# tensorlayer/HyperPose

Hardware: AMD Instinct MI355X
Metric: end-to-end FPS (preproc+DNN+PAF parse) @ 368x432 (higher is better)
Workload: dtype f32; 1 GPU; configs[1]: Lightweight-OpenPose (MobilenetDilated) + PAF parser, batch 8 @ 368x432 per GPU; frames from pinned host memory (one H2D per batch), parser on the network's own maps, humans to the host; key=configs[1]/f32, global_batch=8, parallelism=frame-sharded x1, no steady-state collective, pipes_per_gpu=4, parser_input=the network's own heat-maps

## Files before the change

hyperpose_amd/csrc/conv32_winograd.hip:

```cpp
#include "conv_fp32.hpp"

#include "conv32_epilogue.hpp"
#include "conv_device.hpp"

#include <cstdlib>
#include <vector>

namespace hp {

namespace {

typedef float f32x4 __attribute__((ext_vector_type(4)));
typedef __attribute__((address_space(1))) float gfloat;
typedef __attribute__((address_space(1))) f32x4 gf32x4;

constexpr int WCK = 16;
constexpr int HALO_W = 10;
constexpr int RAW_PB = WCK * 4;
constexpr int VP = 24 * 4;

template <int MW, int NC = 2>
struct wino_geom {
    static constexpr int NT = 64 * MW;
    static constexpr int TB = 4 * NC;
    static constexpr int HALO_H = 8 * NC + 2;
    static constexpr int PATCH_H = HALO_H + 1;
    static constexpr int RAW_Q = PATCH_H * HALO_W * 4;
    static constexpr int NQ = (RAW_Q + NT - 1) / NT;
    static constexpr int RAW_BYTES = NQ * NT * 16;
    static constexpr int NI = 4 * NC / MW;
    static_assert(NI >= 1, "a transform item per wavefront");
    static constexpr int TMS = MW / 2;
    static constexpr int SLAB_PITCH = rows_geom<TMS>::PITCH, SLAB_BYTES = 64 * NC * SLAB_PITCH * 4;
    static constexpr int VPOS = 16 * NC * VP, VBUF = 16 * VPOS;
    static constexpr int LDS_BYTES = RAW_BYTES + (VBUF > SLAB_BYTES ? VBUF : SLAB_BYTES);
    static constexpr int PVPOS = 16 * NC * 64, PVBUF = 16 * PVPOS;
    static constexpr int PLDS_BYTES = RAW_BYTES + (2 * PVBUF > SLAB_BYTES ? 2 * PVBUF : SLAB_BYTES);
};

__device__ __forceinline__ long tvw_off(const tview32& t, int b, int y, int x)
{
    return ((long)b * t.img + (long)y * t.wp + x) * t.cs + t.coff;
}

}

template <int MW, bool PIPE, int NC = 2>
__global__ __launch_bounds__(64 * MW, MW == 8 ? 1 : NC == 1 ? 3 : 2) void conv32_winograd_kernel(const conv32_params p, int tiles_x, int tiles_y, int vh, int T)
{
    static_assert(!PIPE || MW == 4, "the pipelined form is the four-wavefront one");
    using G = wino_geom<MW, NC>;
    constexpr int NT = G::NT, NQ = G::NQ, SLAB_PITCH = G::SLAB_PITCH, VPOS = G::VPOS;
    extern __shared__ __attribute__((aligned(16))) unsigned char lds[];
    unsigned char* const raw = lds;
    unsigned char* const vb = lds + G::RAW_BYTES;

    const int tid = threadIdx.x, lane = tid & 63, wave = tid >> 6;
    const int NG = p.Cout_pad / (16 * MW), ntiles = tiles_x * tiles_y * (vh || T ? 1 : p.B);
    const int Hin = vh ? (p.B - 1) * vh + p.H : p.H;
    const int bj = blockIdx.x >> 3, by = bj % NG;
    int t = (bj / NG) * 8 + (blockIdx.x & 7);
    if (t >= ntiles)
        return;
    const int bx = t;
    const int tx = t % tiles_x;
    t /= tiles_x;
    const int ty = t % tiles_y, b = t / tiles_y;
    const int y0 = ty * (8 * NC), x0 = tx * 8;
    const int MT = p.Cout_pad / 16, mt = by * MW + wave;
    const int nch = p.Cin / WCK;
    int dbg_i = 0;
#define HP_STAMP()                                                     \
    if (p.dbg && bx == 1 && by == 0 && tid == 0)       \
        p.dbg[dbg_i++] = __builtin_amdgcn_s_memtime();
    HP_STAMP();
    if (p.dbg && bx == 1 && by == 0 && tid == 0)
        p.dbg[119] = __builtin_readcyclecounter(), p.dbg[120] = __builtin_amdgcn_s_memrealtime();

    int kb = G::TB, sh = 0, img0 = b, ly0 = y0 - 1, l0 = 0;
    if (T) {
        const int r0 = ty * G::TB;
        img0 = r0 / T, l0 = r0 - img0 * T, ly0 = 2 * l0 - 1;
        kb = min(T - l0, G::TB), sh = kb < G::TB && !(p.H & 1);
    }
    const int Hlim = T ? p.H : Hin, ylow = kb < G::TB ? 2 * kb + 1 + sh : G::PATCH_H;
    const int nvalid = (G::HALO_H + sh) * HALO_W * 4;
    long goff[NQ];
    bool qok[NQ];
#pragma unroll
    for (int i = 0; i < NQ; ++i) {
        const int q = min(tid + i * NT, nvalid - 1);
        const int hp = q >> 2, c4 = q & 3;
        const int hy = hp / HALO_W, hx = hp - hy * HALO_W;
        const bool below = hy >= ylow;
        const int bi = below ? img0 + 1 : img0, y = below ? hy - ylow : ly0 + hy, x = x0 - 1 + hx;
        qok[i] = y <= Hlim && x <= p.W && bi < p.B;
        goff[i] = tvw_off(p.in, min(bi, p.B - 1), min(y, Hlim), min(x, p.W)) + c4 * 4;
    }
    f32x4 stage[NQ];
    auto gload = [&](int c) {
#pragma unroll
        for (int i = 0; i < NQ; ++i)
            stage[i] = *reinterpret_cast<const f32x4*>(p.in.p + goff[i] + min(c, nch - 1) * WCK);
    };
    auto to_lds = [&]() {
#pragma unroll
        for (int i = 0; i < NQ; ++i)
            *reinterpret_cast<f32x4*>(raw + (tid + i * NT) * 16) = qok[i] ? stage[i] : f32x4{ 0.f, 0.f, 0.f, 0.f };
    };
    auto tile_src = [&](int tile, int quad) {
        const int tr = tile >> 2;
        return raw + ((2 * tr + (tr >= kb ? sh : 0)) * HALO_W + 2 * (tile & 3)) * RAW_PB + quad * 16;
    };
    auto transform = [&]() {
#pragma unroll
        for (int k = 0; k < G::NI; ++k) {
            const int item = wave + k * MW, i = NC == 2 ? item >> 1 : item;
            const int quad = lane >> 4, tile = (NC == 2 ? (item & 1) * 16 : 0) + (lane & 15);
            const int ra = i == 0 ? 0 : i == 2 ? 2 : 1, rb = i == 0 ? 2 : i == 1 ? 2 : i == 2 ? 1 : 3;
            const float sg = i == 1 ? 1.f : -1.f;
            const unsigned char* const src = tile_src(tile, quad);
            f32x4 Td[4];
#pragma unroll
            for (int j = 0; j < 4; ++j) {
                const f32x4 a = *reinterpret_cast<const f32x4*>(src + (ra * HALO_W + j) * RAW_PB);
                const f32x4 bq = *reinterpret_cast<const f32x4*>(src + (rb * HALO_W + j) * RAW_PB);
                Td[j] = a + sg * bq;
            }
            constexpr int PS = PIPE ? G::PVPOS : VPOS;
            unsigned char* const dst = PIPE ? vb + (i * 4) * PS + tile * 64 + ((quad ^ ((4 - (tile >> 2)) & 3)) * 16) : vb + (i * 4) * PS + tile * VP + quad * 16;
            *reinterpret_cast<f32x4*>(dst) = Td[0] - Td[2];
            *reinterpret_cast<f32x4*>(dst + PS) = Td[1] + Td[2];
            *reinterpret_cast<f32x4*>(dst + 2 * PS) = Td[2] - Td[1];
            *reinterpret_cast<f32x4*>(dst + 3 * PS) = Td[1] - Td[3];
        }
    };
    f32x4 ta[4], tb[4];
    auto transform_piece = [&](int pos, int buf) {
        const int k = pos >> 3, ps = pos & 7;
        if (k >= G::NI)
            return;
        const int item = wave + k * MW, i = NC == 2 ? item >> 1 : item;
        const int quad = lane >> 4, tile = (NC == 2 ? (item & 1) * 16 : 0) + (lane & 15);
        const int ra = i == 0 ? 0 : i == 2 ? 2 : 1, rb = i == 0 ? 2 : i == 1 ? 2 : i == 2 ? 1 : 3;
        const unsigned char* const src = tile_src(tile, quad);
        if (ps < 4) {
            ta[ps] = *reinterpret_cast<const f32x4*>(src + (ra * HALO_W + ps) * RAW_PB);
            tb[ps] = *reinterpret_cast<const f32x4*>(src + (rb * HALO_W + ps) * RAW_PB);
        } else {
            if (ps == 4) {
                const float sg = i == 1 ? 1.f : -1.f;
#pragma unroll
                for (int j = 0; j < 4; ++j)
                    ta[j] = ta[j] + sg * tb[j];
            }
            unsigned char* const dst = vb + buf * G::PVBUF + (i * 4 + (ps - 4)) * G::PVPOS + tile * 64 + ((quad ^ ((4 - (tile >> 2)) & 3)) * 16);
            *reinterpret_cast<f32x4*>(dst) = ps == 4 ? ta[0] - ta[2] : ps == 5 ? ta[1] + ta[2] : ps == 6 ? ta[2] - ta[1] : ta[1] - ta[3];
        }
    };

    const long step_stride = (long)MT * 256;
    const float* const wp = p.w_wino + (long)mt * 256 + lane * 4;
    const int nsteps = nch * 16;
    constexpr int RING = PIPE ? 4 : 8, AHEAD = PIPE ? 3 : 6;
    f32x4 fa[RING];
    auto aload = [&](int slot, int s) { fa[slot] = *reinterpret_cast<const f32x4*>(wp + (long)min(s, nsteps - 1) * step_stride); };

    f32x4 acc[16][NC];
#pragma unroll
    for (int i = 0; i < 16; ++i)
#pragma unroll
        for (int nc = 0; nc < NC; ++nc)
            acc[i][nc] = f32x4{ 0.f, 0.f, 0.f, 0.f };

    const int btile = lane & 15, kq = lane >> 4;
    const unsigned char* const vsrc = PIPE ? vb + btile * 64 + ((kq ^ ((4 - (btile >> 2)) & 3)) * 16) : vb + btile * VP + kq * 16;
    constexpr int BPOS = PIPE ? G::PVPOS : VPOS, BNT = PIPE ? 16 * 64 : 16 * VP;

    gload(0);
    if constexpr (PIPE) {
#pragma unroll
        for (int a = 0; a < AHEAD; ++a)
            aload(a, a);
        to_lds();
        gload(1);
        lds_barrier();
        HP_STAMP();
        transform();
        lds_barrier();
        to_lds();
        gload(2);
        lds_barrier();
        HP_STAMP();
    } else {
#pragma unroll
        for (int a = 0; a < AHEAD; ++a)
            aload(a, a);
    }
    int s = 0;
#pragma unroll 1
    for (int c = 0; c < nch; ++c) {
        if constexpr (!PIPE) {
            to_lds();
            gload(c + 1);
            lds_barrier();
            HP_STAMP();
            transform();
            lds_barrier();
            HP_STAMP();
        }
        const unsigned char* const vcur = vsrc + (PIPE ? (c & 1) * G::PVBUF : 0);
        f32x4 fb[2][NC];
#pragma unroll
        for (int nc = 0; nc < NC; ++nc)
            fb[0][nc] = *reinterpret_cast<const f32x4*>(vcur + nc * BNT);
#pragma unroll
        for (int pos = 0; pos < 16; ++pos) {
            const int cur = pos & 1, npos = pos + 1 < 16 ? pos + 1 : pos;
#pragma unroll
            for (int nc = 0; nc < NC; ++nc)
                fb[cur ^ 1][nc] = *reinterpret_cast<const f32x4*>(vcur + npos * BPOS + nc * BNT);
            aload((pos + AHEAD) % RING, s + AHEAD);
            const int slot = pos % RING;
#pragma unroll
            for (int e = 0; e < 4; ++e)
#pragma unroll
                for (int nc = 0; nc < NC; ++nc)
                    acc[pos][nc] = __builtin_amdgcn_mfma_f32_16x16x4f32(fa[slot][e], fb[cur][nc][e], acc[pos][nc], 0, 0, 0);
            if constexpr (PIPE)
                transform_piece(pos, (c + 1) & 1);
            __builtin_amdgcn_sched_group_barrier(0x008, 1, 0);
            __builtin_amdgcn_sched_group_barrier(0x100, 1, 0);
            if constexpr (NC == 2) {
                __builtin_amdgcn_sched_group_barrier(0x008, 1, 0);
                __builtin_amdgcn_sched_group_barrier(0x100, 1, 0);
            }
            __builtin_amdgcn_sched_group_barrier(0x008, 1, 0);
            __builtin_amdgcn_sched_group_barrier(0x020, 1, 0);
            __builtin_amdgcn_sched_group_barrier(0x008, NC == 2 ? 5 : 2, 0);
            __builtin_amdgcn_sched_barrier(0);
            ++s;
        }
        HP_STAMP();
        if constexpr (PIPE) {
            if (c + 1 < nch) {
                lds_barrier();
                to_lds();
                gload(c + 3);
                lds_barrier();
                HP_STAMP();
            }
        }
    }

    int tid_o = tid;
    asm volatile("" : "+v"(tid_o));
    const int lane_o = tid_o & 63, btile_o = lane_o & 15, kq_o = lane_o >> 4;
    using R = rows_geom<G::TMS>;
    constexpr int RPW = 64 * NC / MW, NPASS = RPW / R::RPP;
    static_assert(RPW % R::RPP == 0, "slab rows per pass");
    const int dc4 = lane_o % R::LPR, dm = by * 16 * MW + dc4 * 4;
    const bool dany = dm < p.Cout, quads = (p.Cout & 3) == 0;
    const bool out_vec = quads && ((p.out.coff | p.out.cs) & 3) == 0, res_vec = quads && ((p.res.coff | p.res.cs) & 3) == 0;
    const int dmc = dany ? dm : 0;
    int dpix[NPASS], rpix[NPASS];
    bool dok[NPASS];
#pragma unroll
    for (int k = 0; k < NPASS; ++k) {
        const int rr = wave * RPW + k * R::RPP + lane_o / R::LPR, ab = rr / (16 * NC), tile = rr % (16 * NC), tr = tile >> 2;
        const int ox = x0 + 2 * (tile & 3) + (ab & 1);
        int oy, ob;
        if (T)
            ob = tr >= kb ? img0 + 1 : img0, oy = 2 * (tr >= kb ? tr - kb : l0 + tr) + (ab >> 1);
        else {
            oy = y0 + 2 * tr + (ab >> 1);
            ob = vh ? oy / vh : b, oy -= vh ? ob * vh : 0;
        }
        dok[k] = oy < p.OH && ox < p.OW && ob < p.B && dany;
        const int oyc = min(oy, p.OH - 1), oxc = min(ox, p.OW - 1), obc = min(ob, p.B - 1);
        dpix[k] = (obc * p.out.img + oyc * p.out.wp) + oxc;
        rpix[k] = (obc * p.res.img + oyc * p.res.wp) + oxc;
    }
    f32x4 dres[NPASS];
#pragma unroll
    for (int k = 0; k < NPASS; ++k)
        dres[k] = f32x4{ 0.f, 0.f, 0.f, 0.f };
    const gfloat* const gres = (const gfloat*)p.res.p;
    gfloat* const gout = (gfloat*)p.out.p;
    if (gres) {
        if (res_vec) {
#pragma unroll
            for (int k = 0; k < NPASS; ++k)
                dres[k] = *reinterpret_cast<const gf32x4*>(gres + ((long)rpix[k] * p.res.cs + p.res.coff + dmc));
        } else {
#pragma unroll
            for (int k = 0; k < NPASS; ++k)
#pragma unroll
                for (int e = 0; e < 4; ++e)
                    dres[k][e] = gres[(long)rpix[k] * p.res.cs + p.res.coff + min(dm + e, p.Cout - 1)];
        }
    }
    const f32x4 dbs = *(const gf32x4*)(p.bias + dm);
    f32x4 dsl = { p.act_slope, p.act_slope, p.act_slope, p.act_slope };
    if (p.alpha)
        dsl = *(const gf32x4*)(p.alpha + dm);
    lds_barrier();
    HP_STAMP();
    float* const slab = reinterpret_cast<float*>(vb);
#pragma unroll
    for (int nt = 0; nt < NC; ++nt) {
        f32x4 S[2][4];
#pragma unroll
        for (int j = 0; j < 4; ++j) {
            S[0][j] = acc[j][nt] + acc[4 + j][nt] + acc[8 + j][nt];
            S[1][j] = acc[4 + j][nt] - acc[8 + j][nt] - acc[12 + j][nt];
        }
#pragma unroll
        for (int a = 0; a < 2; ++a) {
            const f32x4 y0v = S[a][0] + S[a][1] + S[a][2], y1v = S[a][1] - S[a][2] - S[a][3];
            *reinterpret_cast<f32x4*>(slab + ((a * 2 + 0) * (16 * NC) + nt * 16 + btile_o) * SLAB_PITCH + wave * 16 + kq_o * 4) = y0v;
            *reinterpret_cast<f32x4*>(slab + ((a * 2 + 1) * (16 * NC) + nt * 16 + btile_o) * SLAB_PITCH + wave * 16 + kq_o * 4) = y1v;
        }
    }
    HP_STAMP();
    lds_barrier();
    HP_STAMP();
    const float* const wslab = slab + (wave * RPW + lane_o / R::LPR) * SLAB_PITCH + dc4 * 4;
    f32x4 dv[NPASS];
#pragma unroll
    for (int k = 0; k < NPASS; ++k)
        dv[k] = *reinterpret_cast<const f32x4*>(wslab + k * R::RPP * SLAB_PITCH);
#pragma unroll
    for (int k = 0; k < NPASS; ++k) {
        f32x4 o;
#pragma unroll
        for (int e = 0; e < 4; ++e) {
            float x = dv[k][e] + dbs[e];
            if (p.res.p && p.res_before_act)
                x += dres[k][e];
            x = x > 0.f ? fminf(x, p.act_hi) : x * dsl[e];
            if (p.res.p && !p.res_before_act)
                x += dres[k][e];
            o[e] = x;
        }
        dv[k] = o;
    }
    if (out_vec) {
#pragma unroll
        for (int k = 0; k < NPASS; ++k)
            if (dok[k])
                *reinterpret_cast<gf32x4*>(gout + ((long)dpix[k] * p.out.cs + p.out.coff + dm)) = dv[k];
    } else {
#pragma unroll
        for (int k = 0; k < NPASS; ++k)
#pragma unroll
            for (int e = 0; e < 4; ++e)
                if (dok[k] && dm + e < p.Cout)
                    gout[(long)dpix[k] * p.out.cs + p.out.coff + dm + e] = dv[k][e];
    }
    HP_STAMP();
#undef HP_STAMP
    if (p.dbg && bx == 1 && by == 0 && tid == 0)
        p.dbg[121] = __builtin_readcyclecounter(), p.dbg[122] = __builtin_amdgcn_s_memrealtime();
}

bool conv32_winograd_ok(const conv32_params& p)
{
    return p.KH == 3 && p.KW == 3 && p.stride == 1 && p.dil == 1 && p.Cin % WCK == 0 && p.Cout_pad % 64 == 0 && p.OH == p.H && p.OW == p.W && p.pad_t == 1
        && p.pad_l == 1 && !p.out_f32 && p.out.p;
}

int conv32_winograd_tile(const conv32_params& p) { return p.w_wino3 ? conv32_winograd3_tile(p) : 35000000 + 3000 + 4; }

double conv32_winograd_flops(const conv32_params& p)
{
    return 2.0 * 16 * (double)p.B * ((p.OH + 1) / 2) * ((p.OW + 1) / 2) * p.Cout * p.Cin;
}

void conv32_winograd_pack(const float* packed, int cout_pad, int cin, float* out)
{
    static const double G[4][3] = { { 1, 0, 0 }, { .5, .5, .5 }, { .5, -.5, .5 }, { 0, 0, 1 } };
    const int nch = cin / WCK, MT = cout_pad / 16;
    std::vector<double> U((size_t)16 * cout_pad * cin);
    for (int m = 0; m < cout_pad; ++m)
        for (int k = 0; k < cin; ++k) {
            double g[3][3], Gg[4][3];
            for (int t = 0; t < 9; ++t)
                g[t / 3][t % 3] = packed[((size_t)t * cout_pad + m) * cin + k];
            for (int i = 0; i < 4; ++i)
                for (int j = 0; j < 3; ++j)
                    Gg[i][j] = G[i][0] * g[0][j] + G[i][1] * g[1][j] + G[i][2] * g[2][j];
            for (int i = 0; i < 4; ++i)
                for (int j = 0; j < 4; ++j)
                    U[((size_t)(i * 4 + j) * cout_pad + m) * cin + k] = Gg[i][0] * G[j][0] + Gg[i][1] * G[j][1] + Gg[i][2] * G[j][2];
        }
    for (int c = 0; c < nch; ++c)
        for (int pos = 0; pos < 16; ++pos)
            for (int mt = 0; mt < MT; ++mt) {
                float* dst = out + (((size_t)c * 16 + pos) * MT + mt) * 256;
                for (int lane = 0; lane < 64; ++lane)
                    for (int e = 0; e < 4; ++e) {
                        const int m = mt * 16 + (lane & 15), k = c * WCK + (lane >> 4) * 4 + e;
                        dst[lane * 4 + e] = (float)U[((size_t)pos * cout_pad + m) * cin + k];
                    }
            }
}

template <int MW, bool PIPE, int NC = 2>
static hipError_t launch_wino_case(const conv32_params& q, dim3 grid, int tiles_x, int tiles_y, int vh, int rows, hipStream_t s)
{
    constexpr int lds = PIPE ? wino_geom<MW, NC>::PLDS_BYTES : wino_geom<MW, NC>::LDS_BYTES;
    static bool granted = false;
    if (lds > 64 * 1024 && !granted) {
        const hipError_t e = hipFuncSetAttribute((const void*)conv32_winograd_kernel<MW, PIPE, NC>, hipFuncAttributeMaxDynamicSharedMemorySize, lds);
        if (e != hipSuccess)
            return e;
        granted = true;
    }
    HP_LAUNCH((conv32_winograd_kernel<MW, PIPE, NC>), grid, dim3(64 * MW), lds, s, q, tiles_x, tiles_y, vh, rows);
    return hipGetLastError();
}

static int winograd_nc(const conv32_params& p, const engine_switches& sw, int blocks_nc2)
{
    const int force = sw.wino_nc;
    if (force == 1 || force == 2)
        return force;
    return p.latency && blocks_nc2 <= 512 ? 1 : 2;
}

static int winograd_tall(const conv32_params& p, const engine_switches& sw)
{
    if (!sw.wino_tall)
        return 0;
    if (p.B < 2 || p.in.wp <= 0 || p.in.img % p.in.wp)
        return 0;
    const int vh = p.in.img / p.in.wp;
    return (vh & 1) == 0 && vh >= p.H + 2 ? vh : 0;
}

hipError_t launch_conv32_winograd(const conv32_params& p, const engine_switches& sw, hipStream_t s)
{
    if (!conv32_winograd_ok(p) || !p.w_wino || p.npix <= 0)
        return hipErrorInvalidValue;
    constexpr int mw = 4;
    const int tiles_x = (p.OW + 7) / 8;
    const int nc = winograd_nc(p, sw, tiles_x * ((p.OH + 15) / 16) * p.B * (p.Cout_pad / 64)), bh = 8 * nc;
    int tiles_y = (p.OH + bh - 1) / bh, vh = winograd_tall(p, sw), images = p.B, rows = 0;
    const int T = (p.OH + 1) / 2, rows_y = (p.B * T + 4 * nc - 1) / (4 * nc);
    if (sw.wino_tall && p.B > 1 && T >= 4 * nc && rows_y < tiles_y * p.B)
        tiles_y = rows_y, images = 1, rows = T, vh = 0;
    else if (vh) {
        const int tall_y = ((p.B - 1) * vh + p.H + bh - 1) / bh;
        if (tall_y < tiles_y * p.B)
            tiles_y = tall_y, images = 1;
        else
            vh = 0;
    }
    const dim3 grid((tiles_x * tiles_y * images + 7) / 8 * 8 * (p.Cout_pad / (16 * mw)));
    if (nc == 1)
        return launch_wino_case<4, true, 1>(p, grid, tiles_x, tiles_y, vh, rows, s);
    return launch_wino_case<4, true>(p, grid, tiles_x, tiles_y, vh, rows, s);
}

hipError_t conv32_winograd_occupancy(const conv32_params&, int* blocks_per_cu)
{
    return hipOccupancyMaxActiveBlocksPerMultiprocessor(blocks_per_cu, conv32_winograd_kernel<4, true>, 256, wino_geom<4>::PLDS_BYTES);
}

}
```

hyperpose_amd/csrc/engine.cpp:

```cpp
#include "conv_fp32.hpp"
#include "conv_i8.hpp"
#include "conv_kernels.hpp"
#include "engine_timeline.hpp"
#include "graph_cache.hpp"
#include "hp_common.hpp"
#include "weight_pack.hpp"

#include <algorithm>
#include <cmath>
#include <map>
#include <memory>
#include <string>
#include <variant>
#include <cstdio>
#include <cstdlib>
#include <vector>

namespace {

inline int round_up(int a, int b) { return (a + b - 1) / b * b; }

struct tensor_info {
    bool defined = false;
    bool elided = false;
// ... 1646 lines not shown
bool hp_engine::timeline_of(const step& st, const launch_payload& b, hp::timeline_kind& kind, hp::timeline_header& hd) const
{
    hd = hp::timeline_header{};
    hd.layer = st.layer;
    switch (st.kind) {
    case launch_kind::conv16: {
        const auto& c = std::get<conv16_launch>(b);
        if (c.i8 || !switches.dbg_conv || hp::conv_mfma_tile(c.cp) / 100000 != 52)
            return false;
        kind = hp::timeline_kind::conv, hd.cin = c.cp.Cin, hd.cout = c.cp.Cout, hd.tile = hp::conv_mfma_tile(c.cp);
        return true;
    }
    case launch_kind::bneck:
        kind = hp::timeline_kind::bneck, hd.tile = hp::bottleneck_variant(std::get<hp::bneck_params>(b));
        return switches.dbg_bn;
    case launch_kind::chain:
        kind = hp::timeline_kind::chain, hd.tile = hp::conv_chain_variant(std::get<hp::chain_params>(b));
        return switches.dbg_chain;
    case launch_kind::sep:
        kind = hp::timeline_kind::sep, hd.cin = std::get<hp::sep_params>(b).C;
        return switches.dbg_sep;
    case launch_kind::conv32:
    case launch_kind::wino2:
    case launch_kind::wino3:
    case launch_kind::direct: {
        const hp::conv32_params& q = std::get<conv32_launch>(b).cp;
        if (!switches.dbg_direct || (st.kind == launch_kind::conv32 && q.Cin < switches.dbg_min_cin))
            return false;
        kind = st.kind == launch_kind::conv32 ? hp::timeline_kind::conv32
            : st.kind == launch_kind::wino2   ? hp::timeline_kind::wino
            : st.kind == launch_kind::wino3   ? hp::timeline_kind::wino3
                                              : hp::timeline_kind::direct;
        hd.cin = q.Cin, hd.cout = q.Cout, hd.kh = q.KH, hd.kw = q.KW, hd.tile = tile_of(st.kind, b);
        if (st.kind == launch_kind::wino2)
            (void)hp::conv32_winograd_occupancy(q, &hd.blocks_per_cu);
        return true;
    }
    default: return false;
    }
}

int hp_engine::trace_step(const step& st, launch_payload& b, hipStream_t s) const
{
    hp::timeline_kind kind;
    hp::timeline_header hd;
    if (!timeline_of(st, b, kind, hd))
        return HP_OK;
    const size_t words = hp::timeline_words(kind);
    hp::dev_buf buf;
    HP_TRY(buf.alloc(words * 8));
    HP_HIP_TRY(hipMemset(buf.p, 0, words * 8));
    HP_TRY(launch(st.kind, b, s, buf.as<unsigned long long>()));
    HP_HIP_TRY(hipStreamSynchronize(s));
    std::vector<unsigned long long> hv(words);
    HP_HIP_TRY(hipMemcpy(hv.data(), buf.p, words * 8, hipMemcpyDeviceToHost));
    hp::print_timeline(stderr, kind, hd, hv.data());
    return HP_OK;
}

int hp_engine::run_step(const step& st, const uint8_t* u8, const float* f32, int n, hipStream_t s, int b0) const
{
    launch_payload b = bound(st, u8, f32, n, b0);
    HP_TRY(launch(st.kind, b, s, nullptr));
    return trace_step(st, b, s);
}

int hp_engine::launch_head_pair32(size_t i, int n, int b0, hipStream_t s, bool* done) const
{
    *done = false;
    if (i + 1 >= steps.size() || steps[i].kind != launch_kind::head32 || steps[i + 1].kind != launch_kind::head32)
        return HP_OK;
    const auto &ha = steps[i].as<head32_launch>(), &hb = steps[i + 1].as<head32_launch>();
    const hp::conv32_params a = bind(ha.cp, n, b0), b = bind(hb.cp, n, b0);
    if (!hp::conv32_head_pair_ok(a, b, switches))
        return HP_OK;
    HP_HIP_TRY(hp::launch_conv32_head_pair(a, ha.hh, b, hb.hh, s));
    *done = true;
    return HP_OK;
}

int hp_engine::enqueue_range(const uint8_t* u8, const float* f32, int b0, int n, hipStream_t s) const
{
    for (size_t i = 0; i < steps.size(); ++i) {
        bool paired = false;
        HP_TRY(launch_head_pair32(i, n, b0, s, &paired));
        if (paired)
            ++i;
        else
            HP_TRY(run_step(steps[i], u8, f32, n, s, b0));
    }
    for (auto& o : outputs)
        if (o.fused_layer < 0) {
            const tensor_info& ti = *tensors[o.tensor];
            float* const dst = o.buf->as<float>() + (size_t)b0 * o.out_c() * o.x.out_h * o.x.out_w;
            if (is_f32())
                HP_HIP_TRY(hp::launch_output_transform32(at_frame(ti.view32(o.coff), b0), n, o.H, o.W, o.x, dst, s));
            else
                HP_HIP_TRY(hp::launch_output_transform(ti.view(o.coff), n, o.H, o.W, o.x, dst, s));
        }
    return HP_OK;
}

void hp_engine::fill_row(hp_layer_time* out, int k, int cap, const step& st, int n, float ms) const
{
    if (!out || k >= cap)
        return;
    out[k].layer = st.layer, out[k].op = st.op;
    out[k].tile = step_tile(st, n);
    out[k].ms = ms;
    out[k].flops = st.flops * n, out[k].bytes = st.bytes * n;
}

int hp_engine::stage_profile_input()
{
    const size_t need = (size_t)max_batch * in_h * in_w * 3 * sizeof(float);
    if (in_stage.bytes < need)
        HP_TRY(in_stage.alloc(need));
    return HP_OK;
}

int hp_engine::enqueue(const uint8_t* u8, const float* f32, int n, hipStream_t s, const void* host_src, size_t frame_bytes) const
{
    unsigned char* const dev_in = u8 ? (unsigned char*)u8 : (unsigned char*)f32;
    auto h2d = [&](int b0, int cnt, hipStream_t st) -> int {
        if (host_src)
            HP_HIP_TRY(hipMemcpyAsync(dev_in + (size_t)b0 * frame_bytes, (const unsigned char*)host_src + (size_t)b0 * frame_bytes, (size_t)cnt * frame_bytes, hipMemcpyHostToDevice, st));
        return HP_OK;
    };
    if (parts < 2 || !halves_ok() || n < 2) {
        HP_TRY(h2d(0, n, s));
        return enqueue_range(u8, f32, 0, n, s);
    }
    const int n0 = (n + 1) / 2;
    HP_HIP_TRY(hipEventRecord(ev_fork, s));
    HP_HIP_TRY(hipStreamWaitEvent(stream2, ev_fork, 0));
    HP_TRY(h2d(0, n0, s));
    HP_TRY(h2d(n0, n - n0, stream2));
    HP_TRY(enqueue_range(u8, f32, 0, n0, s));
    HP_TRY(enqueue_range(u8, f32, n0, n - n0, stream2));
    HP_HIP_TRY(hipEventRecord(ev_join, stream2));
    HP_HIP_TRY(hipStreamWaitEvent(s, ev_join, 0));
    return HP_OK;
}

hp::engine_switches hp::read_engine_switches()
{
    auto on = [](const char* name) { return getenv(name) != nullptr; };
    auto num = [](const char* name, int unset) { const char* v = getenv(name); return v ? atoi(v) : unset; };
    engine_switches w;
    w.no_fuse = on("HP_NO_FUSE"), w.no_fuse_head = num("HP_NO_FUSE_HEAD", 0) != 0, w.no_splitk = on("HP_NO_SPLITK");
    w.no_chain = on("HP_NO_CHAIN"), w.no_bneck = on("HP_NO_BNECK"), w.no_seppair = on("HP_NO_SEPPAIR"), w.no_pair_heads = on("HP_NO_PAIR_HEADS");
    w.fuse32 = on("HP_FUSE32"), w.no_fuse32 = on("HP_NO_FUSE32"), w.no_head32 = on("HP_NO_HEAD32"), w.no_arena = on("HP_NO_ARENA");
    w.no_winograd32 = on("HP_NO_WINOGRAD32"), w.wino_f33 = num("HP_WINO_F33", 0) == 1, w.wino_tall = num("HP_WINO_TALL", 1) != 0;
    w.wino_nc = num("HP_WINO_NC", 0), w.head_pair32 = num("HP_HEAD_PAIR", 1) != 0;
    w.c32_wk = num("HP_C32_WK", -1), w.c32_bn160 = num("HP_C32_BN160", -1), w.dw32_px = num("HP_DW32_PX", 0);
    w.lane_epilogue = num("HP_LANE_EPILOGUE", 0), w.first_conv_verify = on("HP_FIRST_CONV_VERIFY");
    w.dbg_conv = on("HP_CONV_DBG"), w.dbg_bn = on("HP_BN_DBG"), w.dbg_chain = on("HP_CHAIN_DBG"), w.dbg_sep = on("HP_SEP_DBG");
    w.dbg_direct = on("HP_DIRECT_DBG"), w.dbg_min_cin = num("HP_DIRECT_DBG_MINCIN", 256);
    return w;
}

extern "C" {

int hp_engine_create(hp_engine** out, const hp_engine_desc* desc)
{
    HP_REQUIRE(out && desc, HP_ERR_INVALID, "hp_engine_create: null argument");
    std::unique_ptr<hp_engine> e(new hp_engine());
    e->switches = hp::read_engine_switches();
    try {
        HP_TRY(e->build(desc));
    } catch (const std::exception& ex) {
        HP_REQUIRE(false, HP_ERR_INVALID, "hp_engine_create: %s", ex.what());
    }
    *out = e.release();
    return HP_OK;
}

namespace {
constexpr char ENGINE_MAGIC[8] = { 'H', 'P', 'E', 'N', 'G', '0', '0', '3' };
struct engine_file_header {
    char magic[8];
    int32_t layer_size, output_size;
    int32_t in_w, in_h, max_batch, flip_rb;
    double factor;
    float mean[3], inv_std[3];
    int32_t n_layers, n_outputs;
    uint64_t n_weights;
    int32_t dtype;
    int32_t n_scales;
};
}

int hp_engine_save(const hp_engine* e, const char* path)
{
    HP_REQUIRE(e && path, HP_ERR_INVALID, "hp_engine_save: null argument");
    FILE* f = fopen(path, "wb");
    HP_REQUIRE(f, HP_ERR_INVALID, "hp_engine_save: cannot open %s for writing", path);
    engine_file_header h{};
    memcpy(h.magic, ENGINE_MAGIC, 8);
    h.layer_size = (int32_t)sizeof(hp_layer), h.output_size = (int32_t)sizeof(hp_output_desc);
    h.in_w = e->in_w, h.in_h = e->in_h, h.max_batch = e->max_batch, h.flip_rb = e->flip_rb, h.factor = e->factor;
    for (int c = 0; c < 3; ++c)
        h.mean[c] = e->mean[c], h.inv_std[c] = e->inv_std[c];
    h.n_layers = (int32_t)e->layers.size(), h.n_outputs = (int32_t)e->out_descs.size(), h.n_weights = e->weights_blob.size();
    h.dtype = e->dtype;
    h.n_scales = (int32_t)e->i8_scale.size();
    bool ok = fwrite(&h, sizeof(h), 1, f) == 1;
    ok = ok && fwrite(e->layers.data(), sizeof(hp_layer), e->layers.size(), f) == e->layers.size();
    ok = ok && fwrite(e->out_descs.data(), sizeof(hp_output_desc), e->out_descs.size(), f) == e->out_descs.size();
    ok = ok && fwrite(e->weights_blob.data(), sizeof(float), e->weights_blob.size(), f) == e->weights_blob.size();
    ok = ok && fwrite(e->i8_scale.data(), sizeof(float), e->i8_scale.size(), f) == e->i8_scale.size();
    ok = (fclose(f) == 0) && ok;
    HP_REQUIRE(ok, HP_ERR_INVALID, "hp_engine_save: short write to %s", path);
    return HP_OK;
}

int hp_engine_load(hp_engine** out, const char* path, int max_batch)
{
    HP_REQUIRE(out && path, HP_ERR_INVALID, "hp_engine_load: null argument");
    FILE* f = fopen(path, "rb");
    HP_REQUIRE(f, HP_ERR_INVALID, "hp_engine_load: cannot open %s", path);
    engine_file_header h{};
    std::vector<hp_layer> layers;
    std::vector<hp_output_desc> outs;
    std::vector<float> w, scales;
    constexpr size_t HDR_001 = offsetof(engine_file_header, dtype);
    bool ok = fread(&h, HDR_001, 1, f) == 1;
    if (ok && memcmp(h.magic, "HPENG001", 8) == 0)
        memcpy(h.magic, ENGINE_MAGIC, 8), h.dtype = HP_DTYPE_F16, h.n_scales = 0;
    else {
        ok = ok && fread(reinterpret_cast<char*>(&h) + HDR_001, sizeof(h) - HDR_001, 1, f) == 1;
        if (ok && memcmp(h.magic, "HPENG002", 8) == 0)
            memcpy(h.magic, ENGINE_MAGIC, 8), ok = h.n_scales == 0 && h.dtype != HP_DTYPE_I8;
    }
    ok = ok && memcmp(h.magic, ENGINE_MAGIC, 8) == 0 && h.layer_size == (int32_t)sizeof(hp_layer)
        && h.output_size == (int32_t)sizeof(hp_output_desc) && h.n_layers > 0 && h.n_layers < (1 << 20) && h.n_outputs > 0
        && h.n_outputs < 4096 && h.n_weights < ((uint64_t)1 << 34)
        && (h.dtype == HP_DTYPE_F16 || h.dtype == HP_DTYPE_F32 || h.dtype == HP_DTYPE_F32S || h.dtype == HP_DTYPE_I8)
        && h.n_scales == (h.dtype == HP_DTYPE_I8 ? h.n_layers : 0);
    if (ok) {
        const long at = ftell(f);
        ok = fseek(f, 0, SEEK_END) == 0;
        const long size = ftell(f);
        ok = ok && fseek(f, at, SEEK_SET) == 0
            && (uint64_t)size == (uint64_t)at + (uint64_t)h.n_layers * sizeof(hp_layer) + (uint64_t)h.n_outputs * sizeof(hp_output_desc) + h.n_weights * sizeof(float)
                    + (uint64_t)h.n_scales * sizeof(float);
    }
    if (ok) {
        layers.resize(h.n_layers), outs.resize(h.n_outputs), w.resize(h.n_weights), scales.resize(h.n_scales);
        ok = fread(layers.data(), sizeof(hp_layer), layers.size(), f) == layers.size()
            && fread(outs.data(), sizeof(hp_output_desc), outs.size(), f) == outs.size() && fread(w.data(), sizeof(float), w.size(), f) == w.size()
            && fread(scales.data(), sizeof(float), scales.size(), f) == scales.size();
    }
    fclose(f);
    HP_REQUIRE(ok, HP_ERR_INVALID, "hp_engine_load: %s is not an engine file written by this library version", path);
    hp_engine_desc d{};
    d.in_w = h.in_w, d.in_h = h.in_h, d.max_batch = max_batch > 0 ? max_batch : h.max_batch, d.factor = h.factor, d.flip_rb = h.flip_rb;
    for (int c = 0; c < 3; ++c)
        d.mean[c] = h.mean[c], d.inv_std[c] = h.inv_std[c];
    d.layers = layers.data(), d.n_layers = h.n_layers, d.outputs = outs.data(), d.n_outputs = h.n_outputs, d.weights = w.data(), d.n_weights = w.size();
    d.dtype = h.dtype;
    d.int8_scales = scales.empty() ? nullptr : scales.data();
    return hp_engine_create(out, &d);
}

void hp_engine_destroy(hp_engine* e)
{
    if (!e)
        return;
    (void)hipDeviceSynchronize();
    delete e;
}

int hp_engine_max_batch(const hp_engine* e) { return e ? e->max_batch : HP_ERR_INVALID; }

int hp_engine_describe(const hp_engine* e, hp_engine_desc* d)
{
    HP_REQUIRE(e && d, HP_ERR_INVALID, "hp_engine_describe: null argument");
    d->in_w = e->in_w, d->in_h = e->in_h, d->max_batch = e->max_batch, d->factor = e->factor, d->flip_rb = e->flip_rb;
    for (int c = 0; c < 3; ++c)
        d->mean[c] = e->mean[c], d->inv_std[c] = e->inv_std[c];
    d->layers = e->layers.data(), d->n_layers = (int32_t)e->layers.size();
    d->outputs = e->out_descs.data(), d->n_outputs = (int32_t)e->out_descs.size();
    d->weights = e->weights_blob.data(), d->n_weights = e->weights_blob.size();
    d->dtype = e->dtype;
    d->int8_scales = e->dtype == HP_DTYPE_I8 ? e->i8_scale.data() : nullptr;
    return HP_OK;
}

int hp_engine_dtype(const hp_engine* e) { return e ? e->dtype : HP_ERR_INVALID; }

int hp_engine_input_size(const hp_engine* e, int* w, int* h)
{
    HP_REQUIRE(e && w && h, HP_ERR_INVALID, "hp_engine_input_size: null argument");
    *w = e->in_w, *h = e->in_h;
    return HP_OK;
}

int hp_engine::leave_split()
{
    HP_TRY(drop_graphs());
    split_off = true, ++split_fallbacks;
    *static_cast<volatile unsigned*>(ovf_flag.p) = 0;
    return HP_OK;
}

static int infer_common(hp_engine* e, const void* input, size_t frame_bytes, int n, int on_device, void* stream, int kind)
// ... 494 lines not shown
```

hyperpose_amd/csrc/hp_common.hpp:

```cpp
#pragma once
#include <hip/hip_runtime.h>

#include <cstdarg>
#include <cstdio>
#include <cstring>
#include <string>
#include <vector>

#include "../../include/hp_hip.h"

namespace hp {

void set_error(const char* fmt, ...) __attribute__((format(printf, 1, 2)));
const char* last_error();

#define HP_HIP_TRY(expr)                                                                                     \
    do {                                                                                                     \
        hipError_t _e = (expr);                                                                              \
        if (_e != hipSuccess) {                                                                              \
            ::hp::set_error("%s failed: %s (%s:%d)", #expr, hipGetErrorString(_e), __FILE__, __LINE__);      \
            return HP_ERR_HIP;                                                                               \
        }                                                                                                    \
    } while (0)

#define HP_REQUIRE(cond, code, ...)                                                                          \
    do {                                                                                                     \
        if (!(cond)) {                                                                                       \
            ::hp::set_error(__VA_ARGS__);                                                                    \
            return (code);                                                                                   \
        }                                                                                                    \
    } while (0)

#define HP_TRY(expr)                                                                                         \
    do {                                                                                                     \
        int _rc = (expr);                                                                                    \
        if (_rc != HP_OK)                                                                                    \
            return _rc;                                                                                      \
    } while (0)

struct dev_buf {
    void* p = nullptr;
    size_t bytes = 0;
    dev_buf() = default;
    dev_buf(const dev_buf&) = delete;
    dev_buf& operator=(const dev_buf&) = delete;
    ~dev_buf() { release(); }
    int alloc(size_t n)
    {
        release();
        if (n == 0)
            return HP_OK;
        HP_HIP_TRY(hipMalloc(&p, n));
        bytes = n;
        return HP_OK;
    }
    void release()
    {
        if (p)
            (void)hipFree(p);
        p = nullptr;
        bytes = 0;
    }
    template <typename T>
    T* as() const { return static_cast<T*>(p); }
};

struct host_buf {
    void* p = nullptr;
    size_t bytes = 0;
    host_buf() = default;
    host_buf(const host_buf&) = delete;
    host_buf& operator=(const host_buf&) = delete;
    ~host_buf() { release(); }
    int alloc(size_t n)
    {
        release();
        if (n == 0)
            return HP_OK;
        HP_HIP_TRY(hipHostMalloc(&p, n, hipHostMallocDefault));
        bytes = n;
        return HP_OK;
    }
    void release()
    {
        if (p)
            (void)hipHostFree(p);
        p = nullptr;
        bytes = 0;
    }
    template <typename T>
    T* as() const { return static_cast<T*>(p); }
};

inline int ceil_div(int a, int b) { return (a + b - 1) / b; }

int merge_humans(const hp_human* in, const int32_t* region_of, int n, int frame_w, int frame_h, int min_common, double tol, std::vector<hp_human>& kept);

struct engine_switches {
    bool no_fuse = false;
    bool no_fuse_head = false;
    bool no_splitk = false;
    bool no_chain = false;
    bool no_bneck = false;
    bool no_seppair = false;
    bool no_pair_heads = false;
    bool fuse32 = false;
    bool no_fuse32 = false;
    bool no_head32 = false;
    bool no_arena = false;
    bool no_winograd32 = false;
    bool wino_f33 = false;
    bool wino_tall = true;
    int wino_nc = 0;
    bool head_pair32 = true;
    int c32_wk = -1;
    int c32_bn160 = -1;
    int dw32_px = 0;
    int lane_epilogue = 0;
    bool first_conv_verify = false;
    bool dbg_conv = false, dbg_bn = false, dbg_chain = false, dbg_sep = false;
    bool dbg_direct = false;
    int dbg_min_cin = 256;
};
engine_switches read_engine_switches();

class frame_pool {
public:
    static frame_pool& instance();
    int workers() const { return n_threads_ + 1; }
    void run(int n_frames, void (*fn)(int frame, int worker, void* ctx), void* ctx);
    ~frame_pool();

private:
    frame_pool();
    struct impl;
    impl* d_;
    int n_threads_;
};

}
```

Baseline: 5482 frames/s.

## Stage Winograd input halo via global_load_lds DMA directly into LDS

Adds a DMA variant of the pipelined fp32 Winograd conv kernel. It loads input halo patches straight into LDS with global_load_lds_dwordx4 instead of going through registers, reschedules the transform around a hand-over point, and uses explicit vmcnt waits for the filter ring. The intent is to drop the register staging and the to_lds stores so that input fetch overlaps the MFMA loop, and to cut VGPR pressure. The change is on by default when channel offsets are aligned. It adds fragile inline asm with m0 manipulation and hand-counted waitcnt values, which risks subtle hazards.

```diff
diff --git a/hyperpose_amd/csrc/conv32_winograd.hip b/hyperpose_amd/csrc/conv32_winograd.hip
--- a/hyperpose_amd/csrc/conv32_winograd.hip
+++ b/hyperpose_amd/csrc/conv32_winograd.hip
@@ -45,10 +45,11 @@
 
 }
 
-template <int MW, bool PIPE, int NC = 2>
-__global__ __launch_bounds__(64 * MW, MW == 8 ? 1 : NC == 1 ? 3 : 2) void conv32_winograd_kernel(const conv32_params p, int tiles_x, int tiles_y, int vh, int T)
+template <int MW, bool PIPE, int NC, bool DMA>
+__device__ __forceinline__ void winograd_block(const conv32_params p, int tiles_x, int tiles_y, int vh, int T)
 {
     static_assert(!PIPE || MW == 4, "the pipelined form is the four-wavefront one");
+    static_assert(!DMA || PIPE, "the LDS-DMA staging belongs to the pipelined form");
     using G = wino_geom<MW, NC>;
     constexpr int NT = G::NT, NQ = G::NQ, SLAB_PITCH = G::SLAB_PITCH, VPOS = G::VPOS;
     extern __shared__ __attribute__((aligned(16))) unsigned char lds[];
@@ -95,8 +96,20 @@
         const bool below = hy >= ylow;
         const int bi = below ? img0 + 1 : img0, y = below ? hy - ylow : ly0 + hy, x = x0 - 1 + hx;
         qok[i] = y <= Hlim && x <= p.W && bi < p.B;
-        goff[i] = tvw_off(p.in, min(bi, p.B - 1), min(y, Hlim), min(x, p.W)) + c4 * 4;
-    }
+        goff[i] = tvw_off(p.in, min(bi, p.B - 1), bi < p.B ? min(y, Hlim) : Hlim, min(x, p.W)) + c4 * 4;
+    }
+    const unsigned raw_lds = __builtin_amdgcn_readfirstlane((unsigned)(size_t)(__attribute__((address_space(3))) unsigned char*)raw + (tid >> 6) * 1024);
+    auto dma = [&](int c) {
+        const float* const src = p.in.p + min(c, nch - 1) * WCK;
+#pragma unroll
+        for (int i = 0; i < NQ; ++i) {
+            unsigned keep;
+            asm volatile("s_mov_b32 %0, m0\n\ts_mov_b32 m0, %2\n\ts_nop 0\n\tglobal_load_lds_dwordx4 %1, off\n\ts_mov_b32 m0, %0"
+                         : "=&s"(keep)
+                         : "v"(src + goff[i]), "s"(raw_lds + i * NT * 16)
+                         : "memory");
+        }
+    };
     f32x4 stage[NQ];
     auto gload = [&](int c) {
 #pragma unroll
@@ -112,7 +125,7 @@
         const int tr = tile >> 2;
         return raw + ((2 * tr + (tr >= kb ? sh : 0)) * HALO_W + 2 * (tile & 3)) * RAW_PB + quad * 16;
     };
-    auto transform = [&]() {
+    auto transform_rows = [&](f32x4 (&Td)[G::NI][4]) {
 #pragma unroll
         for (int k = 0; k < G::NI; ++k) {
             const int item = wave + k * MW, i = NC == 2 ? item >> 1 : item;
@@ -120,20 +133,31 @@
             const int ra = i == 0 ? 0 : i == 2 ? 2 : 1, rb = i == 0 ? 2 : i == 1 ? 2 : i == 2 ? 1 : 3;
             const float sg = i == 1 ? 1.f : -1.f;
             const unsigned char* const src = tile_src(tile, quad);
-            f32x4 Td[4];
 #pragma unroll
             for (int j = 0; j < 4; ++j) {
                 const f32x4 a = *reinterpret_cast<const f32x4*>(src + (ra * HALO_W + j) * RAW_PB);
                 const f32x4 bq = *reinterpret_cast<const f32x4*>(src + (rb * HALO_W + j) * RAW_PB);
-                Td[j] = a + sg * bq;
-            }
+                Td[k][j] = a + sg * bq;
+            }
+        }
+    };
+    auto transform_store = [&](const f32x4 (&Td)[G::NI][4]) {
+#pragma unroll
+        for (int k = 0; k < G::NI; ++k) {
+            const int item = wave + k * MW, i = NC == 2 ? item >> 1 : item;
+            const int quad = lane >> 4, tile = (NC == 2 ? (item & 1) * 16 : 0) + (lane & 15);
             constexpr int PS = PIPE ? G::PVPOS : VPOS;
             unsigned char* const dst = PIPE ? vb + (i * 4) * PS + tile * 64 + ((quad ^ ((4 - (tile >> 2)) & 3)) * 16) : vb + (i * 4) * PS + tile * VP + quad * 16;
-            *reinterpret_cast<f32x4*>(dst) = Td[0] - Td[2];
-            *reinterpret_cast<f32x4*>(dst + PS) = Td[1] + Td[2];
-            *reinterpret_cast<f32x4*>(dst + 2 * PS) = Td[2] - Td[1];
-            *reinterpret_cast<f32x4*>(dst + 3 * PS) = Td[1] - Td[3];
-        }
+            *reinterpret_cast<f32x4*>(dst) = Td[k][0] - Td[k][2];
+            *reinterpret_cast<f32x4*>(dst + PS) = Td[k][1] + Td[k][2];
+            *reinterpret_cast<f32x4*>(dst + 2 * PS) = Td[k][2] - Td[k][1];
+            *reinterpret_cast<f32x4*>(dst + 3 * PS) = Td[k][1] - Td[k][3];
+        }
+    };
+    auto transform = [&]() {
+        f32x4 Td[G::NI][4];
+        transform_rows(Td);
+        transform_store(Td);
     };
     f32x4 ta[4], tb[4];
     auto transform_piece = [&](int pos, int buf) {
@@ -158,13 +182,45 @@
             *reinterpret_cast<f32x4*>(dst) = ps == 4 ? ta[0] - ta[2] : ps == 5 ? ta[1] + ta[2] : ps == 6 ? ta[2] - ta[1] : ta[1] - ta[3];
         }
     };
+    constexpr int HAND = 8;
+    f32x4 qa, qb, ua[4];
+    auto transform_piece_dma = [&](int pos, int buf) {
+#pragma unroll
+        for (int k = 0; k < G::NI; ++k) {
+            const int j = pos - 4 * k;
+            if (j < 0 || j > 7)
+                continue;
+            const int item = wave + k * MW, i = NC == 2 ? item >> 1 : item;
+            const int quad = lane >> 4, tile = (NC == 2 ? (item & 1) * 16 : 0) + (lane & 15);
+            const int ra = i == 0 ? 0 : i == 2 ? 2 : 1, rb = i == 0 ? 2 : i == 1 ? 2 : i == 2 ? 1 : 3;
+            const float sg = i == 1 ? 1.f : -1.f;
+            f32x4* const t = k ? ua : ta;
+            if (j >= 1 && j <= 4)
+                t[j - 1] = qa + sg * qb;
+            if (j < 4) {
+                const unsigned char* const src = tile_src(tile, quad);
+                qa = *reinterpret_cast<const f32x4*>(src + (ra * HALO_W + j) * RAW_PB);
+                qb = *reinterpret_cast<const f32x4*>(src + (rb * HALO_W + j) * RAW_PB);
+            } else {
+                unsigned char* const dst = vb + buf * G::PVBUF + (i * 4 + (j - 4)) * G::PVPOS + tile * 64 + ((quad ^ ((4 - (tile >> 2)) & 3)) * 16);
+                *reinterpret_cast<f32x4*>(dst) = j == 4 ? t[0] - t[2] : j == 5 ? t[1] + t[2] : j == 6 ? t[2] - t[1] : t[1] - t[3];
+            }
+        }
+    };
+    static_assert(4 * (G::NI - 1) + 3 < HAND, "the last patch read comes before the hand-over");
 
     const long step_stride = (long)MT * 256;
     const float* const wp = p.w_wino + (long)mt * 256 + lane * 4;
     const int nsteps = nch * 16;
     constexpr int RING = PIPE ? 4 : 8, AHEAD = PIPE ? 3 : 6;
     f32x4 fa[RING];
-    auto aload = [&](int slot, int s) { fa[slot] = *reinterpret_cast<const f32x4*>(wp + (long)min(s, nsteps - 1) * step_stride); };
+    auto aload = [&](int slot, int s) {
+        const float* const src = wp + (long)min(s, nsteps - 1) * step_stride;
+        if constexpr (DMA)
+            asm volatile("global_load_dwordx4 %0, %1, off" : "=v"(fa[slot]) : "v"(src));
+        else
+            fa[slot] = *reinterpret_cast<const f32x4*>(src);
+    };
 
     f32x4 acc[16][NC];
 #pragma unroll
@@ -177,8 +233,24 @@
     const unsigned char* const vsrc = PIPE ? vb + btile * 64 + ((kq ^ ((4 - (btile >> 2)) & 3)) * 16) : vb + btile * VP + kq * 16;
     constexpr int BPOS = PIPE ? G::PVPOS : VPOS, BNT = PIPE ? 16 * 64 : 16 * VP;
 
-    gload(0);
-    if constexpr (PIPE) {
+    if constexpr (DMA) {
+        dma(0);
+#pragma unroll
+        for (int a = 0; a < AHEAD; ++a)
+            aload(a, a);
+        asm volatile("s_waitcnt vmcnt(%0)" ::"n"(AHEAD) : "memory");
+        lds_barrier();
+        HP_STAMP();
+        f32x4 Td[G::NI][4];
+        transform_rows(Td);
+        lds_barrier();
+        dma(1);
+        transform_store(Td);
+        asm volatile("s_waitcnt vmcnt(0)" ::: "memory");
+        lds_barrier();
+        HP_STAMP();
+    } else if constexpr (PIPE) {
+        gload(0);
 #pragma unroll
         for (int a = 0; a < AHEAD; ++a)
             aload(a, a);
@@ -193,6 +265,7 @@
         lds_barrier();
         HP_STAMP();
     } else {
+        gload(0);
 #pragma unroll
         for (int a = 0; a < AHEAD; ++a)
             aload(a, a);
@@ -217,17 +290,32 @@
 #pragma unroll
         for (int pos = 0; pos < 16; ++pos) {
             const int cur = pos & 1, npos = pos + 1 < 16 ? pos + 1 : pos;
+            if constexpr (DMA)
+                if (pos == HAND) {
+                    lds_barrier();
+                    dma(c + 2);
+                }
 #pragma unroll
             for (int nc = 0; nc < NC; ++nc)
                 fb[cur ^ 1][nc] = *reinterpret_cast<const f32x4*>(vcur + npos * BPOS + nc * BNT);
-            aload((pos + AHEAD) % RING, s + AHEAD);
             const int slot = pos % RING;
+            if constexpr (DMA) {
+                if (pos >= HAND && pos < HAND + AHEAD)
+                    asm volatile("s_waitcnt vmcnt(%1)" : "+v"(fa[slot]) : "n"(AHEAD - 1 + NQ));
+                else
+                    asm volatile("s_waitcnt vmcnt(%1)" : "+v"(fa[slot]) : "n"(AHEAD - 1));
+            } else
+                aload((pos + AHEAD) % RING, s + AHEAD);
 #pragma unroll
             for (int e = 0; e < 4; ++e)
 #pragma unroll
                 for (int nc = 0; nc < NC; ++nc)
                     acc[pos][nc] = __builtin_amdgcn_mfma_f32_16x16x4f32(fa[slot][e], fb[cur][nc][e], acc[pos][nc], 0, 0, 0);
-            if constexpr (PIPE)
+            if constexpr (DMA) {
+                aload((pos + AHEAD) % RING, s + AHEAD);
+                transform_piece_dma(pos, (c + 1) & 1);
+            }
+            else if constexpr (PIPE)
                 transform_piece(pos, (c + 1) & 1);
             __builtin_amdgcn_sched_group_barrier(0x008, 1, 0);
             __builtin_amdgcn_sched_group_barrier(0x100, 1, 0);
@@ -242,7 +330,13 @@
             ++s;
         }
         HP_STAMP();
-        if constexpr (PIPE) {
+        if constexpr (DMA) {
+            if (c + 1 < nch) {
+                asm volatile("s_waitcnt vmcnt(%0)" ::"n"(AHEAD) : "memory");
+                lds_barrier();
+                HP_STAMP();
+            }
+        } else if constexpr (PIPE) {
             if (c + 1 < nch) {
                 lds_barrier();
                 to_lds();
@@ -251,6 +345,13 @@
                 HP_STAMP();
             }
         }
+    }
+
+    if constexpr (DMA)
+    {
+#pragma unroll
+        for (int a = 0; a < RING; ++a)
+            asm volatile("s_waitcnt vmcnt(0)" : "+v"(fa[a])::"memory");
     }
 
     int tid_o = tid;
@@ -362,6 +463,18 @@
 #undef HP_STAMP
     if (p.dbg && bx == 1 && by == 0 && tid == 0)
         p.dbg[121] = __builtin_readcyclecounter(), p.dbg[122] = __builtin_amdgcn_s_memrealtime();
+}
+
+template <int MW, bool PIPE, int NC = 2>
+__global__ __launch_bounds__(64 * MW, MW == 8 ? 1 : NC == 1 ? 3 : 2) void conv32_winograd_kernel(const conv32_params p, int tiles_x, int tiles_y, int vh, int T)
+{
+    winograd_block<MW, PIPE, NC, PIPE>(p, tiles_x, tiles_y, vh, T);
+}
+
+template <int MW, bool PIPE, int NC = 2>
+__global__ __launch_bounds__(64 * MW, MW == 8 ? 1 : NC == 1 ? 3 : 2) void conv32_winograd_staged_kernel(const conv32_params p, int tiles_x, int tiles_y, int vh, int T)
+{
+    winograd_block<MW, PIPE, NC, false>(p, tiles_x, tiles_y, vh, T);
 }
 
 bool conv32_winograd_ok(const conv32_params& p)
@@ -406,18 +519,19 @@
             }
 }
 
-template <int MW, bool PIPE, int NC = 2>
+template <int MW, bool PIPE, int NC, bool DMA>
 static hipError_t launch_wino_case(const conv32_params& q, dim3 grid, int tiles_x, int tiles_y, int vh, int rows, hipStream_t s)
 {
     constexpr int lds = PIPE ? wino_geom<MW, NC>::PLDS_BYTES : wino_geom<MW, NC>::LDS_BYTES;
+    constexpr auto kernel = DMA ? conv32_winograd_kernel<MW, PIPE, NC> : conv32_winograd_staged_kernel<MW, PIPE, NC>;
     static bool granted = false;
     if (lds > 64 * 1024 && !granted) {
-        const hipError_t e = hipFuncSetAttribute((const void*)conv32_winograd_kernel<MW, PIPE, NC>, hipFuncAttributeMaxDynamicSharedMemorySize, lds);
+        const hipError_t e = hipFuncSetAttribute((const void*)kernel, hipFuncAttributeMaxDynamicSharedMemorySize, lds);
         if (e != hipSuccess)
             return e;
         granted = true;
     }
-    HP_LAUNCH((conv32_winograd_kernel<MW, PIPE, NC>), grid, dim3(64 * MW), lds, s, q, tiles_x, tiles_y, vh, rows);
+    HP_LAUNCH(kernel, grid, dim3(64 * MW), lds, s, q, tiles_x, tiles_y, vh, rows);
     return hipGetLastError();
 }
 
@@ -458,9 +572,10 @@
             vh = 0;
     }
     const dim3 grid((tiles_x * tiles_y * images + 7) / 8 * 8 * (p.Cout_pad / (16 * mw)));
+    const bool dma = sw.wino_dma && ((p.in.coff | p.in.cs) & 3) == 0;
     if (nc == 1)
-        return launch_wino_case<4, true, 1>(p, grid, tiles_x, tiles_y, vh, rows, s);
-    return launch_wino_case<4, true>(p, grid, tiles_x, tiles_y, vh, rows, s);
+        return dma ? launch_wino_case<4, true, 1, true>(p, grid, tiles_x, tiles_y, vh, rows, s) : launch_wino_case<4, true, 1, false>(p, grid, tiles_x, tiles_y, vh, rows, s);
+    return dma ? launch_wino_case<4, true, 2, true>(p, grid, tiles_x, tiles_y, vh, rows, s) : launch_wino_case<4, true, 2, false>(p, grid, tiles_x, tiles_y, vh, rows, s);
 }
 
 hipError_t conv32_winograd_occupancy(const conv32_params&, int* blocks_per_cu)
diff --git a/hyperpose_amd/csrc/engine.cpp b/hyperpose_amd/csrc/engine.cpp
--- a/hyperpose_amd/csrc/engine.cpp
+++ b/hyperpose_amd/csrc/engine.cpp
@@ -1822,7 +1822,7 @@
     w.no_chain = on("HP_NO_CHAIN"), w.no_bneck = on("HP_NO_BNECK"), w.no_seppair = on("HP_NO_SEPPAIR"), w.no_pair_heads = on("HP_NO_PAIR_HEADS");
     w.fuse32 = on("HP_FUSE32"), w.no_fuse32 = on("HP_NO_FUSE32"), w.no_head32 = on("HP_NO_HEAD32"), w.no_arena = on("HP_NO_ARENA");
     w.no_winograd32 = on("HP_NO_WINOGRAD32"), w.wino_f33 = num("HP_WINO_F33", 0) == 1, w.wino_tall = num("HP_WINO_TALL", 1) != 0;
-    w.wino_nc = num("HP_WINO_NC", 0), w.head_pair32 = num("HP_HEAD_PAIR", 1) != 0;
+    w.wino_nc = num("HP_WINO_NC", 0), w.wino_dma = num("HP_WINO_DMA", 1) != 0, w.head_pair32 = num("HP_HEAD_PAIR", 1) != 0;
     w.c32_wk = num("HP_C32_WK", -1), w.c32_bn160 = num("HP_C32_BN160", -1), w.dw32_px = num("HP_DW32_PX", 0);
     w.lane_epilogue = num("HP_LANE_EPILOGUE", 0), w.first_conv_verify = on("HP_FIRST_CONV_VERIFY");
     w.dbg_conv = on("HP_CONV_DBG"), w.dbg_bn = on("HP_BN_DBG"), w.dbg_chain = on("HP_CHAIN_DBG"), w.dbg_sep = on("HP_SEP_DBG");
diff --git a/hyperpose_amd/csrc/hp_common.hpp b/hyperpose_amd/csrc/hp_common.hpp
--- a/hyperpose_amd/csrc/hp_common.hpp
+++ b/hyperpose_amd/csrc/hp_common.hpp
@@ -111,6 +111,7 @@
     bool no_winograd32 = false;
     bool wino_f33 = false;
     bool wino_tall = true;
+    bool wino_dma = true;
     int wino_nc = 0;
     bool head_pair32 = true;
     int c32_wk = -1;
```

Result: no change. 5519 frames/s, median of 6 (+0.7%).
